# robert80203/HuPR-A-Benchmark-for-Human-Pose-Estimation-Using-Millimeter-Wave-Radar

Measured on AMD Instinct MI355X. Metric: radar frames/sec (FFT->heatmap fwd+bwd), higher is better.
Workload: dtype bf16

## Files before the change

hupr-a-benchmark-for-human-pose-estimation-using-millimeter-wave-radar_amd/csrc/attention_bf16.hip:

```cpp
#include "gemm_common.h"

namespace hupr {

constexpr float kLog2e = 1.4426950408889634f;
constexpr float kLn2 = 0.6931471805599453f;
constexpr float kDeferBits = 8.f;

typedef __bf16 bf16x8 __attribute__((ext_vector_type(8)));
typedef short s16x4 __attribute__((ext_vector_type(4)));

template <int D>
struct Img {
    static constexpr int CH = D / 8;
    static __device__ __forceinline__ int key(int row) {
        return (D == 64) ? ((((row >> 1) & 1) << 2) | ((row >> 2) & 3)) : ((((row & 3) << 2) | ((row >> 2) & 3)) | (row & (D / 8 - 1) & ~15));
    }
    static __device__ __forceinline__ int off(int row, int chunk) { return row * D + ((chunk ^ key(row)) << 3); }
};

typedef unsigned u32x4a __attribute__((ext_vector_type(4)));

template <int D, int ROWS, typename TI>
__device__ __forceinline__ void stage_rows(__bf16* img, const TI* __restrict__ src, long ld, int tid) {
    constexpr int CH = D / 8, ITEMS = ROWS * CH, PER = ITEMS / 256;
// ... 470 lines not shown
    load_frags<D, TI>(qf, Q + ((long)by * N + q) * ldq, lh);
    load_frags<D, TI>(gf, dO + ((long)by * N + q) * lddo, lh);
    const float nlse_q = -lse[(long)by * N + q] * kLog2e, d_q = Dq[(long)by * N + q];
    f32x16 nlse16;
#pragma unroll
    for (int r = 0; r < 16; ++r) nlse16[r] = nlse_q;
    f32x16 dq[D / 32];
#pragma unroll
    for (int ct = 0; ct < D / 32; ++ct)
#pragma unroll
        for (int r = 0; r < 16; ++r) dq[ct][r] = 0.f;
    constexpr bool PF = (D <= 128);
    StageRegs<PF ? D : 64, KT, TI> kr, vr;
    if (PF) {
        kr.load(K, ldk, tid);
        vr.load(V + base, D, tid);
    }
    for (int j0 = 0; j0 < N; j0 += KT) {
        __syncthreads();
        if (PF) {
            kr.store(Ks, tid);
            vr.store(Vs, tid);
        } else {
            stage_rows<D, KT, TI>(Ks, K + (long)j0 * ldk, ldk, tid);
            stage_rows<D, KT, TI>(Vs, V + base + (long)j0 * D, D, tid);
        }
        __syncthreads();
        if (PF && j0 + KT < N) {
            kr.load(K + (long)(j0 + KT) * ldk, ldk, tid);
            vr.load(V + base + (long)(j0 + KT) * D, D, tid);
        }
        f32x16 st[NT], dp[NT];
        if constexpr (QS) {
#pragma unroll
            for (int t = 0; t < NT; ++t) st[t] = nlse16;
            mma_rows_x_frags<D, false, NT>(st, Ks, qf, lr, lh);
        } else {
            mma_rows_x_frags<D, true, NT>(st, Ks, qf, lr, lh);
        }
        mma_rows_x_frags<D, true, NT>(dp, Vs, gf, lr, lh);
        {
            typedef float f32x2a __attribute__((ext_vector_type(2)));
#pragma unroll
            for (int t = 0; t < NT; ++t)
#pragma unroll
                for (int r = 0; r < 16; r += 2) {
                    const f32x2a arg = QS ? (f32x2a){st[t][r], st[t][r + 1]}
                                          : __builtin_elementwise_fma((f32x2a){st[t][r], st[t][r + 1]}, (f32x2a){kLog2e, kLog2e}, (f32x2a){nlse_q, nlse_q});
                    const f32x2a pv = {__builtin_amdgcn_exp2f(arg[0]), __builtin_amdgcn_exp2f(arg[1])};
                    const f32x2a ds = pv * ((f32x2a){dp[t][r], dp[t][r + 1]} - (f32x2a){d_q, d_q});
                    st[t][r] = ds[0];
                    st[t][r + 1] = ds[1];
                }
        }
        mma_tr_x_tile<D, D / 32, NT>(dq, Ks, st, lane);
    }
    store_ct<D>(dQ + ((long)by * N + q) * lddq, dq, 1.f, nullptr, lh);
}

template <int D, typename TI, int NH, bool QS = false>
__global__ __launch_bounds__(256, D == 64 ? 2 : 1) void hupr_k_attn_bwd_dkv(const TI* __restrict__ K, const TI* __restrict__ Q,
                                                           const TI* __restrict__ V, const TI* __restrict__ dO,
                                                           const float* dVadd,
                                                           const float* __restrict__ lse, const float* __restrict__ Dq,
                                                           float* __restrict__ dK, float* dV, int N, int ldk,
                                                           int ldq, int lddk, int lddo, const __bf16* dVadd16, int ldadd16, int xcd_map,
                                                           const AttnBwdBatch batch = AttnBwdBatch()) {
    __shared__ __attribute__((aligned(16))) __bf16 Qs[64 * D];
    __shared__ __attribute__((aligned(16))) __bf16 Gs[64 * D];
    __shared__ __attribute__((aligned(16))) float s_lse[64], s_d[64];
    const int tid = threadIdx.x, lane = tid & 63, wave = tid >> 6, lr = lane & 31, lh = lane >> 5;
    int bx, by;
    xcd_block(bx, by, xcd_map);
    if (batch.n > 0) {
        const int item = by / batch.Bn;
        by -= item * batch.Bn;
        K = static_cast<const TI*>(batch.K[item]);
        Q = static_cast<const TI*>(batch.Q[item]);
        V = static_cast<const TI*>(batch.V[item]);
        dO = static_cast<const TI*>(batch.dO[item]);
        lse = batch.lse[item];
        Dq = batch.Dq[item];
        dK = batch.dK[item];
        dV = batch.dV[item];
        dVadd = batch.add32[item];
        dVadd16 = batch.add16[item];
    }
    const long base = (long)by * N * D;
    const int key = bx * 128 + wave * 32 + lr;
    bf16x8 kf[D / 16], vf[D / 16];
    load_frags<D, TI>(kf, K + ((long)by * N + key) * ldk, lh);
    load_frags<D, TI>(vf, V + base + (long)key * D, lh);
    Q += (long)by * N * ldq;
    dO += (long)by * N * lddo;
    constexpr int DV = D / NH;
    const int c0 = blockIdx.z * DV;
    f32x16 dk[DV / 32], dv[DV / 32];
#pragma unroll
    for (int ct = 0; ct < DV / 32; ++ct)
#pragma unroll
        for (int r = 0; r < 16; ++r) { dk[ct][r] = 0.f; dv[ct][r] = 0.f; }
    constexpr bool PFQ = (D <= 128), PFG = (D == 128);
    StageRegs<PFQ ? D : 64, 64, TI> qr;
    StageRegs<PFG ? D : 64, 64, TI> gr;
    if (PFQ) qr.load(Q, ldq, tid);
    if (PFG) gr.load(dO, lddo, tid);
    for (int q0 = 0; q0 < N; q0 += 64) {
        __syncthreads();
        if (PFQ) qr.store(Qs, tid);
        else stage_rows<D, 64, TI>(Qs, Q + (long)q0 * ldq, ldq, tid);
        if (PFG) gr.store(Gs, tid);
        else stage_rows<D, 64, TI>(Gs, dO + (long)q0 * lddo, lddo, tid);
        if (tid < 64) {
            s_lse[tid] = -lse[(long)by * N + q0 + tid] * kLog2e;
            s_d[tid] = Dq[(long)by * N + q0 + tid];
        }
        __syncthreads();
        if (q0 + 64 < N) {
            if (PFQ) qr.load(Q + (long)(q0 + 64) * ldq, ldq, tid);
            if (PFG) gr.load(dO + (long)(q0 + 64) * lddo, lddo, tid);
        }
        f32x16 s[2], dp[2];
        if constexpr (QS) {
#pragma unroll
            for (int t = 0; t < 2; ++t)
#pragma unroll
                for (int r4 = 0; r4 < 4; ++r4) {
                    const float4 l4 = *reinterpret_cast<const float4*>(&s_lse[32 * t + 8 * r4 + 4 * lh]);
                    s[t][4 * r4] = l4.x; s[t][4 * r4 + 1] = l4.y; s[t][4 * r4 + 2] = l4.z; s[t][4 * r4 + 3] = l4.w;
                }
            mma_rows_x_frags<D, false>(s, Qs, kf, lr, lh);
        } else {
            mma_rows_x_frags<D>(s, Qs, kf, lr, lh);
        }
        mma_rows_x_frags<D>(dp, Gs, vf, lr, lh);
#pragma unroll
        for (int t = 0; t < 2; ++t)
#pragma unroll
            for (int r = 0; r < 16; ++r) {
                const int qi = 32 * t + (r & 3) + 8 * (r >> 2) + 4 * lh;
                const float pv = __builtin_amdgcn_exp2f(QS ? s[t][r] : fmaf(s[t][r], kLog2e, s_lse[qi]));
                dp[t][r] = pv * (dp[t][r] - s_d[qi]);
                s[t][r] = pv;
            }
        mma_tr_x_tile<D, DV / 32>(dv, Gs, s, lane, c0 / 32);
        mma_tr_x_tile<D, DV / 32>(dk, Qs, dp, lane, c0 / 32);
    }
    store_ct<DV>(dK + ((long)by * N + key) * lddk + c0, dk, QS ? kLn2 : 1.f, nullptr, lh);
    if (dVadd16) store_ct_add16<DV>(dV + base + (long)key * D + c0, dv, dVadd16 + ((long)by * N + key) * ldadd16 + c0, lh);
    else store_ct<DV>(dV + base + (long)key * D + c0, dv, 1.f, dVadd ? dVadd + base + (long)key * D + c0 : nullptr, lh);
}


template <bool QS>
__global__ __launch_bounds__(512) void hupr_k_attn_bwd_dkv512(const __bf16* __restrict__ K, const __bf16* __restrict__ Q,
                                                              const __bf16* __restrict__ V, const __bf16* __restrict__ dO,
                                                              const float* dVadd, const float* __restrict__ lse,
                                                              const float* __restrict__ Dq, float* __restrict__ dK, float* dV, int N,
                                                              int ldk, int ldq, int lddk, int lddo, const __bf16* dVadd16,
                                                              int ldadd16, int xcd_map) {
    constexpr int D = 64;
    __shared__ __attribute__((aligned(16))) __bf16 Qs[2][64 * D];
    __shared__ __attribute__((aligned(16))) __bf16 Gs[2][64 * D];
    __shared__ __attribute__((aligned(16))) float s_lse[2][64], s_d[2][64];
    const int tid = threadIdx.x, lane = tid & 63, wave = tid >> 6, lr = lane & 31, lh = lane >> 5;
    int bx, by;
    xcd_block(bx, by, xcd_map);
    const long base = (long)by * N * D;
    const int key = bx * 256 + wave * 32 + lr;
    bf16x8 kf[D / 16], vf[D / 16];
    load_frags<D, __bf16>(kf, K + ((long)by * N + key) * ldk, lh);
    load_frags<D, __bf16>(vf, V + base + (long)key * D, lh);
    Q += (long)by * N * ldq;
    dO += (long)by * N * lddo;
    f32x16 dk[D / 32], dv[D / 32];
#pragma unroll
    for (int ct = 0; ct < D / 32; ++ct)
#pragma unroll
        for (int r = 0; r < 16; ++r) { dk[ct][r] = 0.f; dv[ct][r] = 0.f; }
    const int srow = tid >> 3, sch = tid & 7;
    const __bf16* qp = Q + (long)srow * ldq + sch * 8;
    const __bf16* gp = dO + (long)srow * lddo + sch * 8;
    const float* sp = tid < 64 ? lse + (long)by * N + tid : Dq + (long)by * N + (tid & 63);
    u32x4a qreg = *reinterpret_cast<const u32x4a*>(qp), greg = *reinterpret_cast<const u32x4a*>(gp);
    float sreg = tid < 128 ? *sp : 0.f;
    *reinterpret_cast<u32x4a*>(&Qs[0][Img<D>::off(srow, sch)]) = qreg;
    *reinterpret_cast<u32x4a*>(&Gs[0][Img<D>::off(srow, sch)]) = greg;
    if (tid < 64) s_lse[0][tid] = -sreg * kLog2e;
    else if (tid < 128) s_d[0][tid - 64] = sreg;
    __syncthreads();
    for (int q0 = 0; q0 < N; q0 += 64) {
        const int cb = (q0 >> 6) & 1;
        if (q0 + 64 < N) {
            qreg = *reinterpret_cast<const u32x4a*>(qp + (long)(q0 + 64) * ldq);
            greg = *reinterpret_cast<const u32x4a*>(gp + (long)(q0 + 64) * lddo);
            if (tid < 128) sreg = sp[q0 + 64];
        }
        f32x16 s[2], dp[2];
        if constexpr (QS) {
#pragma unroll
            for (int t = 0; t < 2; ++t)
#pragma unroll
                for (int r4 = 0; r4 < 4; ++r4) {
                    const float4 l4 = *reinterpret_cast<const float4*>(&s_lse[cb][32 * t + 8 * r4 + 4 * lh]);
                    s[t][4 * r4] = l4.x; s[t][4 * r4 + 1] = l4.y; s[t][4 * r4 + 2] = l4.z; s[t][4 * r4 + 3] = l4.w;
                }
            mma_rows_x_frags<D, false>(s, Qs[cb], kf, lr, lh);
        } else {
            mma_rows_x_frags<D>(s, Qs[cb], kf, lr, lh);
        }
        mma_rows_x_frags<D>(dp, Gs[cb], vf, lr, lh);
        typedef float f32x2a __attribute__((ext_vector_type(2)));
#pragma unroll
        for (int t = 0; t < 2; ++t)
#pragma unroll
            for (int r = 0; r < 16; r += 2) {
                const int qi = 32 * t + (r & 3) + 8 * (r >> 2) + 4 * lh;
                const f32x2a dd = *reinterpret_cast<const f32x2a*>(&s_d[cb][qi]);
                f32x2a arg = {s[t][r], s[t][r + 1]};
                if constexpr (!QS) arg = __builtin_elementwise_fma(arg, (f32x2a){kLog2e, kLog2e}, *reinterpret_cast<const f32x2a*>(&s_lse[cb][qi]));
                const f32x2a pv = {__builtin_amdgcn_exp2f(arg[0]), __builtin_amdgcn_exp2f(arg[1])};
                const f32x2a ds = pv * ((f32x2a){dp[t][r], dp[t][r + 1]} - dd);
                dp[t][r] = ds[0];
                dp[t][r + 1] = ds[1];
                s[t][r] = pv[0];
                s[t][r + 1] = pv[1];
            }
        mma_tr_x_tile<D, D / 32>(dv, Gs[cb], s, lane, 0);
        mma_tr_x_tile<D, D / 32>(dk, Qs[cb], dp, lane, 0);
        if (q0 + 64 < N) {
            *reinterpret_cast<u32x4a*>(&Qs[cb ^ 1][Img<D>::off(srow, sch)]) = qreg;
            *reinterpret_cast<u32x4a*>(&Gs[cb ^ 1][Img<D>::off(srow, sch)]) = greg;
            if (tid < 64) s_lse[cb ^ 1][tid] = -sreg * kLog2e;
            else if (tid < 128) s_d[cb ^ 1][tid - 64] = sreg;
        }
        __syncthreads();
    }
    store_ct<D>(dK + ((long)by * N + key) * lddk, dk, QS ? kLn2 : 1.f, nullptr, lh);
    if (dVadd16) store_ct_add16<D>(dV + base + (long)key * D, dv, dVadd16 + ((long)by * N + key) * ldadd16, lh);
    else store_ct<D>(dV + base + (long)key * D, dv, 1.f, dVadd ? dVadd + base + (long)key * D : nullptr, lh);
}

typedef float v2fa __attribute__((ext_vector_type(2)));
constexpr int kPPRing = 8, kPPAhead = 4;

__device__ __forceinline__ void pp_dma(unsigned m0val, int voff, u32x4a rsrc, int soff) {
    unsigned keep;
    m0val = __builtin_amdgcn_readfirstlane(m0val);
    soff = __builtin_amdgcn_readfirstlane(soff);
    asm volatile("s_mov_b32 %0, m0\n\ts_mov_b32 m0, %1\n\ts_nop 0\n\tbuffer_load_dwordx4 %2, %3, %4 offen lds\n\ts_mov_b32 m0, %0"
                 : "=&s"(keep)
                 : "s"(m0val), "v"(voff), "s"(rsrc), "s"(soff)
                 : "memory");
}
#define HUPR_PP_VMCNT(N_) __builtin_amdgcn_s_waitcnt(0x0F70 | ((N_) & 15) | (((N_) >> 4) << 14))
#define HUPR_PP_BARRIER()                    \
    __builtin_amdgcn_sched_barrier(0);       \
    __builtin_amdgcn_s_barrier();            \
    __builtin_amdgcn_sched_barrier(0)

__device__ __forceinline__ u32x4a pp_rsrc(const void* base, long bytes) {
    return (u32x4a){(unsigned)(unsigned long)base, (unsigned)((unsigned long)base >> 32) & 0xffffu, (unsigned)bytes, 0x00020000u};
}

__device__ __forceinline__ void pp_block(int nqb, int Bn, int& b, int& qb) {
    const int L = blockIdx.x;
    if (Bn % 8 == 0) {
        const int idx = L >> 3;
        qb = idx % nqb;
        b = (L & 7) + 8 * (idx / nqb);
    } else {
        qb = L % nqb;
        b = L / nqb;
    }
}

template <bool QS = false>
__global__ __launch_bounds__(512, 1) void hupr_k_attn_fwd_pp64(const __bf16* __restrict__ K, const __bf16* __restrict__ Q,
                                                              const __bf16* __restrict__ V, const float* __restrict__ Vres,
                                                              float* __restrict__ out, float* __restrict__ lse, int N, int Bn, int ldk,
                                                              int ldq, __bf16* __restrict__ out16, int ld16,
                                                              unsigned long long* __restrict__ trace) {
    constexpr int D = 64;
    __shared__ __attribute__((aligned(1024))) __bf16 ring[kPPRing][2][64 * D];
    const bool tracing = trace != nullptr && blockIdx.x == 0 && (threadIdx.x >> 6) % 4 == 0;
    unsigned long long* tr = trace + (threadIdx.x >> 8) * 4096;
    int tslot = 0;
#define HUPR_PP_STAMP()                                                             \
    if (tracing) {                                                                  \
        const unsigned long long t__ = __builtin_amdgcn_s_memtime();                \
        if ((threadIdx.x & 63) == 0 && tslot < 4096) tr[tslot] = t__;               \
        ++tslot;                                                                    \
    }
    const int tid = threadIdx.x, lane = tid & 63, wave = tid >> 6, lr = lane & 31, lh = lane >> 5;
    const int grp = wave >> 2;
    if (grp == 0) __builtin_amdgcn_s_setprio(1);
    int b, qb;
    pp_block(N / 256, Bn, b, qb);
    const long base = (long)b * N * D;
    const int q = qb * 256 + wave * 32 + lr;
    const int nt = N / 64;
    bf16x8 qf[4];
    load_frags<D, __bf16>(qf, Q + ((long)b * N + q) * ldq, lh);

    const int prow = 8 * wave + (lane >> 3);
    const int pchunk = (lane & 7) ^ Img<D>::key(prow);
    const int kvoff = (prow * ldk + pchunk * 8) * 2, vvoff = (prow * D + pchunk * 8) * 2;
    const u32x4a krs = pp_rsrc(K + (long)b * N * ldk, (long)N * ldk * 2), vrs = pp_rsrc(V + base, (long)N * D * 2);
    const unsigned lds0 = (unsigned)(unsigned long)(__attribute__((address_space(3))) void*)&ring[0][0][0];
    const unsigned piece = __builtin_amdgcn_readfirstlane(lds0 + wave * 1024);
#define HUPR_PP_ISSUE(TILE_)                                                                    \
    {                                                                                           \
        const int tl_ = min((TILE_), nt - 1), sl_ = (TILE_) & (kPPRing - 1);                    \
        pp_dma(piece + sl_ * 16384, kvoff, krs, tl_ * 64 * ldk * 2);                            \
        pp_dma(piece + sl_ * 16384 + 8192, vvoff, vrs, tl_ * 64 * D * 2);                       \
    }
    int koff[4];
#pragma unroll
    for (int ks = 0; ks < 4; ++ks) koff[ks] = Img<D>::off(lr, 2 * ks + lh);
    const int g = lane >> 4, s16 = lane & 15, h = g >> 1;
    const int col = 16 * (g & 1) + 4 * (s16 & 3), rsub = s16 >> 2;
    int voff0[2], voff1[2];
#pragma unroll
    for (int ct = 0; ct < 2; ++ct) {
        const int c = 32 * ct + col;
        voff0[ct] = Img<D>::off(4 * h + rsub, c >> 3) + (c & 4);
        voff1[ct] = Img<D>::off(4 * h + rsub + 8, c >> 3) + (c & 4);
    }

    f32x16 o[2], st[2][2];
#pragma unroll
    for (int ct = 0; ct < 2; ++ct)
#pragma unroll
        for (int r = 0; r < 16; ++r) o[ct][r] = 0.f;
    float m_run = QS ? 0.f : -INFINITY, l_run = 0.f;
    f32x16 negm16 = {0.f, 0.f, 0.f, 0.f, 0.f, 0.f, 0.f, 0.f, 0.f, 0.f, 0.f, 0.f, 0.f, 0.f, 0.f, 0.f};
    bf16x8 kf[2][4], vf[2][2][2], pb[2][2][2];

#define HUPR_PP_READ_K(SLOT_)                                                                                      \
    {                                                                                                              \
        const __bf16* ki_ = &ring[SLOT_][0][0];                                                                    \
        _Pragma("unroll") for (int ks = 0; ks < 4; ++ks)                                                           \
            _Pragma("unroll") for (int t = 0; t < 2; ++t)                                                          \
                kf[t][ks] = *reinterpret_cast<const bf16x8*>(ki_ + koff[ks] + t * 32 * D);                         \
    }
#define HUPR_PP_READ_V(SLOT_)                                                                                      \
    {                                                                                                              \
        const __bf16* vi_ = &ring[SLOT_][1][0];                                                                    \
        _Pragma("unroll") for (int t = 0; t < 2; ++t)                                                              \
            _Pragma("unroll") for (int u = 0; u < 2; ++u)                                                          \
                _Pragma("unroll") for (int ct = 0; ct < 2; ++ct) {                                                 \
                    const s16x4 lo_ = __builtin_amdgcn_ds_read_tr16_b64_v4i16(                                     \
                        (__attribute__((address_space(3))) s16x4*)(vi_ + voff0[ct] + (32 * t + 16 * u) * D));     \
                    const s16x4 hi_ = __builtin_amdgcn_ds_read_tr16_b64_v4i16(                                     \
                        (__attribute__((address_space(3))) s16x4*)(vi_ + voff1[ct] + (32 * t + 16 * u) * D));     \
                    union { struct { s16x4 a, b; } s2; bf16x8 v; } uu_;                                            \
                    uu_.s2.a = lo_;                                                                                \
                    uu_.s2.b = hi_;                                                                                \
                    vf[t][u][ct] = uu_.v;                                                                          \
                }                                                                                                  \
    }
#define HUPR_PP_S(DST_)                                                                                            \
    {                                                                                                              \
        _Pragma("unroll") for (int t = 0; t < 2; ++t)                                                              \
            _Pragma("unroll") for (int r = 0; r < 16; ++r) st[DST_][t][r] = 0.f;                                   \
        _Pragma("unroll") for (int ks = 0; ks < 4; ++ks)                                                           \
            _Pragma("unroll") for (int t = 0; t < 2; ++t)                                                          \
                st[DST_][t] = __builtin_amdgcn_mfma_f32_32x32x16_bf16(kf[t][ks], qf[ks], st[DST_][t], 0, 0, 0);    \
    }
#define HUPR_PP_PV(SRC_)                                                                                           \
    _Pragma("unroll") for (int t = 0; t < 2; ++t)                                                                  \
        _Pragma("unroll") for (int u = 0; u < 2; ++u)                                                              \
            _Pragma("unroll") for (int ct = 0; ct < 2; ++ct)                                                       \
                o[ct] = __builtin_amdgcn_mfma_f32_32x32x16_bf16(vf[t][u][ct], pb[SRC_][t][u], o[ct], 0, 0, 0);

    HUPR_PP_ISSUE(0)
    HUPR_PP_ISSUE(1)
    HUPR_PP_ISSUE(2)
    HUPR_PP_ISSUE(3)
    HUPR_PP_VMCNT(4);
    HUPR_PP_BARRIER();
    HUPR_PP_READ_K(0)
    HUPR_PP_S(0)

#define HUPR_SB() __builtin_amdgcn_sched_barrier(0)
#define HUPR_PVM(T_, U_, CT_)                                                                                              \
    if (!(FIRST__)) o[CT_] = __builtin_amdgcn_mfma_f32_32x32x16_bf16(vf[T_][U_][CT_], pb[NXT__][T_][U_], o[CT_], 0, 0, 0);
#define HUPR_SM(KS_, T_)                                                                                                   \
    if (!(LAST__)) {                                                                                        \
        asm volatile("" : "+v"(kf[T_][KS_]));                                                                              \
        if ((KS_) == 0) st[NXT__][T_] = __builtin_amdgcn_mfma_f32_32x32x16_bf16(kf[T_][0], qf[0], QS ? negm16 : zero16, 0, 0, 0); \
        else st[NXT__][T_] = __builtin_amdgcn_mfma_f32_32x32x16_bf16(kf[T_][KS_], qf[KS_], st[NXT__][T_], 0, 0, 0);        \
        asm volatile("" : "+v"(kf[T_][KS_]));                                                                              \
    }
#define HUPR_M3(A_, B_, C_) fmaxf(fmaxf(A_, B_), C_)
#define HUPR_PAIR(P_)                                                                                                      \
    {                                                                                                                      \
        constexpr int t_ = (P_) >> 3, u_ = ((P_) >> 2) & 1, i_ = 2 * ((P_) & 3);                                           \
        v2fa s2_ = {st[CUR__][t_][8 * u_ + i_], st[CUR__][t_][8 * u_ + i_ + 1]};                                           \
        asm volatile("" : "+v"(s2_));                                                                                      \
        const v2fa e2_ = QS ? s2_ : __builtin_elementwise_fma(s2_, l2e2, nm2);                                             \
        const float p0_ = __builtin_amdgcn_exp2f(e2_.x);                                                         \
        const float p1_ = __builtin_amdgcn_exp2f(e2_.y);                                                         \
        sum2[(P_) & 1] += (v2fa){p0_, p1_};                                                                                \
        pb[CUR__][t_][u_][i_] = (__bf16)p0_;                                                                               \
        pb[CUR__][t_][u_][i_ + 1] = (__bf16)p1_;                                                                           \
        if (((P_) & 1) == 1) asm volatile("" : "+v"(sum2[0]), "+v"(sum2[1]));                                              \
    }
    const f32x16 zero16 = {0.f, 0.f, 0.f, 0.f, 0.f, 0.f, 0.f, 0.f, 0.f, 0.f, 0.f, 0.f, 0.f, 0.f, 0.f, 0.f};
#define HUPR_PP_TILE(CUR_, NXT_, FIRST_, LAST_)                                                                            \
    {                                                                                                                      \
        constexpr int CUR__ = CUR_, NXT__ = NXT_;                                                                          \
        constexpr bool FIRST__ = FIRST_, LAST__ = LAST_;                                                                   \
        HUPR_PP_STAMP()                                                                                                    \
        { HUPR_PP_ISSUE(j + kPPAhead) }                                                                           \
        if (!LAST__) { HUPR_PP_READ_K             ((j + 1) & (kPPRing - 1)) }                                             \
        HUPR_SB();                                                                                                         \
                          \
        const f32x16& s0_ = st[CUR__][0];                                                                                  \
        const f32x16& s1_ = st[CUR__][1];                                                                                  \
        float ma_, mb_, mc_, md_;                                                                                          \
        HUPR_PVM(0, 0, 0) ma_ = HUPR_M3(s0_[0], s0_[1], s0_[2]); mb_ = HUPR_M3(s0_[8], s0_[9], s0_[10]); HUPR_SB();        \
        HUPR_PVM(0, 0, 1) mc_ = HUPR_M3(s1_[0], s1_[1], s1_[2]); md_ = HUPR_M3(s1_[8], s1_[9], s1_[10]); HUPR_SB();        \
        HUPR_PVM(0, 1, 0) ma_ = HUPR_M3(ma_, s0_[3], s0_[4]); mb_ = HUPR_M3(mb_, s0_[11], s0_[12]); HUPR_SB();             \
        HUPR_PVM(0, 1, 1) mc_ = HUPR_M3(mc_, s1_[3], s1_[4]); md_ = HUPR_M3(md_, s1_[11], s1_[12]); HUPR_SB();             \
        HUPR_PVM(1, 0, 0) ma_ = HUPR_M3(ma_, s0_[5], s0_[6]); mb_ = HUPR_M3(mb_, s0_[13], s0_[14]); HUPR_SB();             \
        HUPR_PVM(1, 0, 1) mc_ = HUPR_M3(mc_, s1_[5], s1_[6]); md_ = HUPR_M3(md_, s1_[13], s1_[14]); HUPR_SB();             \
// ... 174 lines not shown
            HUPR_PP_FWD();
#undef HUPR_PP_FWD
            HUPR_LAUNCH_OK("hupr_k_attn_fwd_pp64");
            return HUPR_OK;
        }
    }
    if (plan_fwd(route) == HUPR_ATTN_FWD_SPLIT) {
        HUPR_REQUIRE(ws_bytes >= hupr_attn_fwd_split_ws_bytes(Bn, N, C), "%s: workspace too small", who);
        const long rows = (long)Bn * N;
        float* part_o = static_cast<float*>(ws);
        float* part_ml = part_o + (long)S * rows * C;
        grid.z = S;
        const dim3 cgrid((unsigned)((rows * (C / 4) + 255) / 256));
        hipStream_t s = as_stream(stream);
#define HUPR_ATTN_SPLIT(D_)                                                                                                \
        HUPR_LAUNCH((hupr_k_attn_fwd<D_, TI, true, QS>), grid, dim3(256), 0, s, K, Q, V, Vres, out, lse, N, ldk, ldq, o16, ld16, \
                           part_o, part_ml, AttnBatch());                                                                  \
        HUPR_LAUNCH((hupr_k_attn_combine<D_, QS>), cgrid, dim3(256), 0, s, part_o, part_ml, S, rows, Vres, out, lse, o16, ld16, AttnBatch());
        if (C == 64) { HUPR_ATTN_SPLIT(64) } else if (C == 128) { HUPR_ATTN_SPLIT(128) } else { HUPR_ATTN_SPLIT(256) }
#undef HUPR_ATTN_SPLIT
        HUPR_LAUNCH_OK("hupr_k_attn_fwd (split)");
        return HUPR_OK;
    }
    if (C == 64) HUPR_LAUNCH((hupr_k_attn_fwd<64, TI, false, QS>), grid, dim3(256), 0, as_stream(stream), K, Q, V, Vres, out, lse, N, ldk, ldq, o16, ld16, np, np, AttnBatch());
    else if (C == 128) HUPR_LAUNCH((hupr_k_attn_fwd<128, TI, false, QS>), grid, dim3(256), 0, as_stream(stream), K, Q, V, Vres, out, lse, N, ldk, ldq, o16, ld16, np, np, AttnBatch());
    else HUPR_LAUNCH((hupr_k_attn_fwd<256, TI, false, QS>), grid, dim3(256), 0, as_stream(stream), K, Q, V, Vres, out, lse, N, ldk, ldq, o16, ld16, np, np, AttnBatch());
    HUPR_LAUNCH_OK("hupr_k_attn_fwd");
    return HUPR_OK;
}

extern "C" int hupr_attn_fwd_bf16(const float* K, const float* Q, const float* V, float* out, float* lse, int Bn, int N, int C,
                                  int residual, hupr_stream_t stream) {
    return attn_fwd("hupr_attn_fwd_bf16", K, C, Q, C, V, residual ? V : nullptr, out, lse, nullptr, 0, Bn, N, C, stream);
}
extern "C" int hupr_attn_fwd_bf16in(const void* K, const void* Q, const void* V, const float* Vres, float* out, float* lse,
                                    int Bn, int N, int C, hupr_stream_t stream) {
    return attn_fwd("hupr_attn_fwd_bf16in", static_cast<const __bf16*>(K), C, static_cast<const __bf16*>(Q), C,
                    static_cast<const __bf16*>(V), Vres, out, lse, nullptr, 0, Bn, N, C, stream);
}
extern "C" int hupr_attn_fwd_bf16in_ld(const void* K, int ldk, const void* Q, int ldq, const void* V, const float* Vres,
                                       float* out, float* lse, void* out16, int ld16, int Bn, int N, int C,
                                       hupr_stream_t stream) {
    return attn_fwd("hupr_attn_fwd_bf16in_ld", static_cast<const __bf16*>(K), ldk, static_cast<const __bf16*>(Q), ldq,
                    static_cast<const __bf16*>(V), Vres, out, lse, out16, ld16, Bn, N, C, stream);
}
template <bool QS>
static int attn_fwd_batch(const char* who, const hupr_attn_item* items, int n_items, int ldk, int ldq, int ld16, int Bn, int N,
                          int C, void* ws, size_t ws_bytes, hupr_stream_t stream) {
    HUPR_REQUIRE(items && n_items >= 1 && n_items <= 4 && Bn > 0, "%s: bad argument", who);
    HUPR_REQUIRE(hupr_attn_flash_supported(N, C), "%s: unsupported shape N=%d C=%d", who, N, C);
    HUPR_REQUIRE(ldk >= C && ldq >= C && ldk % 8 == 0 && ldq % 8 == 0, "%s: bad row strides %d %d", who, ldk, ldq);
    const int route = attn_plan(Bn, N, C, ldk, true, ws != nullptr);
    HUPR_REQUIRE(route > 0, "%s: bad argument", who);
    const int S = plan_splits(route);
    bool any16 = false;
    for (int i = 0; i < n_items; ++i) {
        HUPR_REQUIRE(items[i].K && items[i].Q && items[i].V && items[i].out && items[i].lse, "%s: null pointer in item %d", who, i);
        any16 = any16 || items[i].out16;
    }
    HUPR_REQUIRE(!any16 || (ld16 >= C && ld16 % 4 == 0), "%s: bad bf16 output stride %d", who, ld16);
    if (plan_fwd(route) == HUPR_ATTN_FWD_PP64) {
        for (int i = 0; i < n_items; ++i) {
            const int rc = attn_fwd<__bf16, QS>(who, static_cast<const __bf16*>(items[i].K), ldk, static_cast<const __bf16*>(items[i].Q), ldq,
                                               static_cast<const __bf16*>(items[i].V), items[i].Vres, items[i].out, items[i].lse,
                                               items[i].out16, ld16, Bn, N, C, stream);
            if (rc) return rc;
        }
        return HUPR_OK;
    }
    HUPR_REQUIRE(S == 1 || ws_bytes >= (size_t)n_items * hupr_attn_fwd_split_ws_bytes(Bn, N, C), "%s: workspace too small", who);
    AttnBatch b = AttnBatch();
    b.n = n_items;
    b.splits = S;
    for (int i = 0; i < n_items; ++i) {
        b.K[i] = items[i].K; b.Q[i] = items[i].Q; b.V[i] = items[i].V; b.Vres[i] = items[i].Vres;
        b.out[i] = items[i].out; b.lse[i] = items[i].lse; b.out16[i] = static_cast<__bf16*>(items[i].out16);
    }
    if (plan_fwd(route) == HUPR_ATTN_FWD_ONE_PASS) {
        const dim3 g1(N / 128, Bn, n_items);
        hipStream_t s1 = as_stream(stream);
        const __bf16* const k0 = nullptr;
        float* const f0 = nullptr;
        __bf16* const h0 = nullptr;
        if (C == 64) HUPR_LAUNCH((hupr_k_attn_fwd<64, __bf16, false, QS>), g1, dim3(256), 0, s1, k0, k0, k0, f0, f0, f0, N, ldk, ldq, h0, ld16, f0, f0, b);
        else if (C == 128) HUPR_LAUNCH((hupr_k_attn_fwd<128, __bf16, false, QS>), g1, dim3(256), 0, s1, k0, k0, k0, f0, f0, f0, N, ldk, ldq, h0, ld16, f0, f0, b);
        else HUPR_LAUNCH((hupr_k_attn_fwd<256, __bf16, false, QS>), g1, dim3(256), 0, s1, k0, k0, k0, f0, f0, f0, N, ldk, ldq, h0, ld16, f0, f0, b);
        HUPR_LAUNCH_OK("hupr_k_attn_fwd (batch)");
        return HUPR_OK;
    }
    const long rows = (long)Bn * N;
    float* part_o = static_cast<float*>(ws);
    float* part_ml = part_o + (long)n_items * S * rows * C;
    const dim3 grid(N / 128, Bn, S * n_items);
    const dim3 cgrid((unsigned)((rows * (C / 4) + 255) / 256), n_items);
    hipStream_t s = as_stream(stream);
    typedef __bf16 TI;
    const TI* const nk = nullptr;
    float* const nf = nullptr;
    __bf16* const nh = nullptr;
#define HUPR_ATTN_BATCH(D_)                                                                                                          \
    HUPR_LAUNCH((hupr_k_attn_fwd<D_, TI, true, QS>), grid, dim3(256), 0, s, nk, nk, nk, nf, nf, nf, N, ldk, ldq, nh, ld16, part_o, part_ml, b); \
    HUPR_LAUNCH((hupr_k_attn_combine<D_, QS>), cgrid, dim3(256), 0, s, part_o, part_ml, S, rows, nf, nf, nf, nh, ld16, b);
    if (C == 64) { HUPR_ATTN_BATCH(64) } else if (C == 128) { HUPR_ATTN_BATCH(128) } else { HUPR_ATTN_BATCH(256) }
#undef HUPR_ATTN_BATCH
    HUPR_LAUNCH_OK("hupr_k_attn_fwd (split, batch)");
    return HUPR_OK;
}
extern "C" int hupr_attn_fwd_bf16in_ld_ws_batch(const hupr_attn_item* items, int n_items, int ldk, int ldq, int ld16, int Bn, int N,
                                                int C, void* ws, size_t ws_bytes, hupr_stream_t stream) {
    return attn_fwd_batch<false>("hupr_attn_fwd_bf16in_ld_ws_batch", items, n_items, ldk, ldq, ld16, Bn, N, C, ws, ws_bytes, stream);
}
extern "C" int hupr_attn_fwd_bf16in_ld_ws_batch_qs(const hupr_attn_item* items, int n_items, int ldk, int ldq, int ld16, int Bn, int N,
                                                   int C, void* ws, size_t ws_bytes, hupr_stream_t stream) {
    return attn_fwd_batch<true>("hupr_attn_fwd_bf16in_ld_ws_batch_qs", items, n_items, ldk, ldq, ld16, Bn, N, C, ws, ws_bytes, stream);
}

extern "C" int hupr_attn_fwd_bf16in_ld_ws(const void* K, int ldk, const void* Q, int ldq, const void* V, const float* Vres,
                                          float* out, float* lse, void* out16, int ld16, int Bn, int N, int C, void* ws,
                                          size_t ws_bytes, hupr_stream_t stream) {
    return attn_fwd("hupr_attn_fwd_bf16in_ld_ws", static_cast<const __bf16*>(K), ldk, static_cast<const __bf16*>(Q), ldq,
                    static_cast<const __bf16*>(V), Vres, out, lse, out16, ld16, Bn, N, C, stream, ws, ws_bytes);
}
extern "C" int hupr_attn_fwd_bf16in_ld_ws_qs(const void* K, int ldk, const void* Qs, int ldq, const void* V, const float* Vres,
                                             float* out, float* lse, void* out16, int ld16, int Bn, int N, int C, void* ws,
                                             size_t ws_bytes, hupr_stream_t stream) {
    return attn_fwd<__bf16, true>("hupr_attn_fwd_bf16in_ld_ws_qs", static_cast<const __bf16*>(K), ldk, static_cast<const __bf16*>(Qs), ldq,
                                  static_cast<const __bf16*>(V), Vres, out, lse, out16, ld16, Bn, N, C, stream, ws, ws_bytes);
}

template <typename TI, bool QS = false>
static int attn_bwd(const char* who, const TI* K, int ldk, const TI* Q, int ldq, const TI* V, const TI* dO, int lddo,
                    const float* V32, const float* out, const float* dout32, const float* lse, float* dK, int lddk, float* dQ,
                    int lddq, float* dV, int accumulate, float* Dq, int Bn, int N, int C, int residual, hupr_stream_t stream) {
    HUPR_REQUIRE(K && Q && V && dO && V32 && out && lse && dK && dQ && dV && Dq && Bn > 0, "%s: bad argument", who);
    HUPR_REQUIRE(dout32 || sizeof(TI) == 2, "%s: fp32 operands need the fp32 gradient", who);
    HUPR_REQUIRE(hupr_attn_flash_supported(N, C), "%s: unsupported shape N=%d C=%d", who, N, C);
    HUPR_REQUIRE(ldk >= C && ldq >= C && lddk >= C && lddq >= C && lddo >= C && ldk % 8 == 0 && ldq % 8 == 0 && lddo % 8 == 0 &&
                     lddk % 4 == 0 && lddq % 4 == 0,
                 "%s: bad row strides", who);
    HUPR_REQUIRE(!(residual && accumulate), "%s: accumulate is for the non-residual form", who);
    const int route = attn_plan(Bn, N, C, ldk, sizeof(TI) == 2, false);
    HUPR_REQUIRE(route > 0, "%s: bad argument", who);
    hipStream_t s = as_stream(stream);
    const long rows = (long)Bn * N;
    dim3 grid(N / 128, Bn);
    const float* add32 = residual ? dout32 : (accumulate ? dV : nullptr);
    const __bf16* add16 = (residual && !dout32) ? reinterpret_cast<const __bf16*>(dO) : nullptr;
    const dim3 pgrid((unsigned)((rows + 15) / 16));
    const int xmap = plan_xmap(route);
    const bool dkv512 = plan_dkv(route) == HUPR_ATTN_DKV512;
#define HUPR_ATTN_BWD(D_, NH_)                                                                                             \
    if (dout32) HUPR_LAUNCH((hupr_k_attn_prep<D_, float>), pgrid, dim3(256), 0, s, dout32, C, out, V32, Dq, rows, residual); \
    else HUPR_LAUNCH((hupr_k_attn_prep<D_, __bf16>), pgrid, dim3(256), 0, s, reinterpret_cast<const __bf16*>(dO), lddo, out, V32, Dq, rows, residual); \
    HUPR_LAUNCH((hupr_k_attn_bwd_dq<D_, TI, QS>), grid, dim3(256), 0, s, K, Q, V, dO, lse, Dq, dQ, N, ldk, ldq, lddq, lddo, xmap);  \
    if (dkv512)                                                                                                              \
        HUPR_LAUNCH(hupr_k_attn_bwd_dkv512<QS>, dim3(N / 256, Bn), dim3(512), 0, s, reinterpret_cast<const __bf16*>(K),       \
                           reinterpret_cast<const __bf16*>(Q), reinterpret_cast<const __bf16*>(V), reinterpret_cast<const __bf16*>(dO), \
                           add32, lse, Dq, dK, dV, N, ldk, ldq, lddk, lddo, add16, lddo, xmap);                                 \
    else                                                                                                                     \
        HUPR_LAUNCH((hupr_k_attn_bwd_dkv<D_, TI, NH_, QS>), dim3(N / 128, Bn, NH_), dim3(256), 0, s, K, Q, V, dO, add32, lse, Dq, \
                           dK, dV, N, ldk, ldq, lddk, lddo, add16, lddo, xmap);
    if (C == 64) { HUPR_ATTN_BWD(64, 1) } else if (C == 128) { HUPR_ATTN_BWD(128, 1) } else { HUPR_ATTN_BWD(256, 2) }
#undef HUPR_ATTN_BWD
    HUPR_LAUNCH_OK("hupr_k_attn_bwd");
    return HUPR_OK;
}

template <bool QS>
static int attn_bwd_batch(const char* who, const hupr_attn_bwd_item* items, int n_items, int ldk, int ldq, int lddo, int lddk, int lddq,
                          int Bn, int N, int C, hupr_stream_t stream) {
    HUPR_REQUIRE(items && n_items >= 1 && n_items <= 4 && Bn > 0, "%s: bad argument", who);
    HUPR_REQUIRE(hupr_attn_flash_supported(N, C), "%s: unsupported shape N=%d C=%d", who, N, C);
    for (int i = 0; i < n_items; ++i) {
        const hupr_attn_bwd_item& t = items[i];
        HUPR_REQUIRE(t.K && t.Q && t.V && t.dO && t.V32 && t.out && t.lse && t.dK && t.dQ && t.dV && t.Dq, "%s: null pointer in item %d", who, i);
        HUPR_REQUIRE(!(t.residual && t.accumulate), "%s: accumulate is for the non-residual form (item %d)", who, i);
    }
    const int route = attn_plan(Bn, N, C, ldk, true, false);
    HUPR_REQUIRE(route > 0, "%s: bad row strides", who);
    const bool level1 = plan_dkv(route) == HUPR_ATTN_DKV512;
    if (n_items == 1) {
        for (int i = 0; i < n_items; ++i) {
            const hupr_attn_bwd_item& t = items[i];
            const int rc = attn_bwd<__bf16, QS>(who, static_cast<const __bf16*>(t.K), ldk, static_cast<const __bf16*>(t.Q), ldq,
                                               static_cast<const __bf16*>(t.V), static_cast<const __bf16*>(t.dO), lddo, t.V32, t.out, nullptr,
                                               t.lse, t.dK, lddk, t.dQ, lddq, t.dV, t.accumulate, t.Dq, Bn, N, C, t.residual, stream);
            if (rc) return rc;
        }
        return HUPR_OK;
    }
    HUPR_REQUIRE(ldk >= C && ldq >= C && lddk >= C && lddq >= C && lddo >= C && ldk % 8 == 0 && ldq % 8 == 0 && lddo % 8 == 0 &&
                     lddk % 4 == 0 && lddq % 4 == 0, "%s: bad row strides", who);
    hipStream_t s = as_stream(stream);
    const long rows = (long)Bn * N;
    const int xmap = plan_xmap(route);
    AttnBwdBatch b = AttnBwdBatch();
    b.n = n_items;
    b.Bn = Bn;
    for (int i = 0; i < n_items; ++i) {
        const hupr_attn_bwd_item& t = items[i];
        b.K[i] = t.K; b.Q[i] = t.Q; b.V[i] = t.V; b.dO[i] = t.dO; b.out[i] = t.out; b.V32[i] = t.V32; b.lse[i] = t.lse;
        b.Dq[i] = t.Dq; b.dK[i] = t.dK; b.dQ[i] = t.dQ; b.dV[i] = t.dV; b.residual[i] = t.residual;
        b.add32[i] = t.accumulate ? t.dV : nullptr;
        b.add16[i] = t.residual ? static_cast<const __bf16*>(t.dO) : nullptr;
    }
    const __bf16* const k0 = nullptr;
    const float* const c0 = nullptr;
    float* const f0 = nullptr;
    const dim3 pgrid((unsigned)((rows + 15) / 16), n_items), qgrid(N / 128, Bn * n_items);
    int round_of[4], n_rounds = 0;
    for (int i = 0; i < n_items; ++i) {
        int r = 0;
        for (int j = 0; j < i; ++j)
            if (items[j].dV == items[i].dV) r = round_of[j] + 1 > r ? round_of[j] + 1 : r;
        round_of[i] = r;
        n_rounds = r + 1 > n_rounds ? r + 1 : n_rounds;
    }
#define HUPR_ATTN_BWD_BATCH(D_, NH_)                                                                                             \
    HUPR_LAUNCH((hupr_k_attn_prep<D_, __bf16>), pgrid, dim3(256), 0, s, k0, lddo, c0, c0, f0, rows, 0, b);                      \
    HUPR_LAUNCH((hupr_k_attn_bwd_dq<D_, __bf16, QS>), qgrid, dim3(256), 0, s, k0, k0, k0, k0, c0, c0, f0, N, ldk, ldq, lddq, lddo, xmap, b); \
    for (int r = 0; r < n_rounds; ++r) {                                                                                         \
        AttnBwdBatch br = AttnBwdBatch();                                                                                        \
        br.Bn = Bn;                                                                                                              \
        for (int i = 0; i < n_items; ++i)                                                                                        \
            if (round_of[i] == r) {                                                                                              \
                const int k = br.n++;                                                                                            \
                br.K[k] = b.K[i]; br.Q[k] = b.Q[i]; br.V[k] = b.V[i]; br.dO[k] = b.dO[i]; br.lse[k] = b.lse[i]; br.Dq[k] = b.Dq[i]; \
                br.dK[k] = b.dK[i]; br.dV[k] = b.dV[i]; br.add32[k] = b.add32[i]; br.add16[k] = b.add16[i];                      \
            }                                                                                                                    \
        HUPR_LAUNCH((hupr_k_attn_bwd_dkv<D_, __bf16, NH_, QS>), dim3(N / 128, Bn * br.n, NH_), dim3(256), 0, s, k0, k0, k0, k0, c0, c0, c0, \
                    f0, f0, N, ldk, ldq, lddk, lddo, k0, lddo, xmap, br);                                                        \
    }
    if (level1) {
        HUPR_LAUNCH((hupr_k_attn_prep<64, __bf16>), pgrid, dim3(256), 0, s, k0, lddo, c0, c0, f0, rows, 0, b);
        HUPR_LAUNCH((hupr_k_attn_bwd_dq<64, __bf16, QS>), qgrid, dim3(256), 0, s, k0, k0, k0, k0, c0, c0, f0, N, ldk, ldq, lddq, lddo, xmap, b);
        for (int i = 0; i < n_items; ++i)
            HUPR_LAUNCH(hupr_k_attn_bwd_dkv512<QS>, dim3(N / 256, Bn), dim3(512), 0, s, static_cast<const __bf16*>(b.K[i]),
                        static_cast<const __bf16*>(b.Q[i]), static_cast<const __bf16*>(b.V[i]), static_cast<const __bf16*>(b.dO[i]), b.add32[i],
                        b.lse[i], b.Dq[i], b.dK[i], b.dV[i], N, ldk, ldq, lddk, lddo, b.add16[i], lddo, xmap);
    } else if (C == 64) { HUPR_ATTN_BWD_BATCH(64, 1) } else if (C == 128) { HUPR_ATTN_BWD_BATCH(128, 1) } else { HUPR_ATTN_BWD_BATCH(256, 2) }
#undef HUPR_ATTN_BWD_BATCH
    HUPR_LAUNCH_OK("hupr_k_attn_bwd (batch)");
    return HUPR_OK;
}
extern "C" int hupr_attn_bwd_bf16in_ld_batch(const hupr_attn_bwd_item* items, int n_items, int ldk, int ldq, int lddo, int lddk,
                                             int lddq, int Bn, int N, int C, hupr_stream_t stream) {
    return attn_bwd_batch<false>("hupr_attn_bwd_bf16in_ld_batch", items, n_items, ldk, ldq, lddo, lddk, lddq, Bn, N, C, stream);
}
extern "C" int hupr_attn_bwd_bf16in_ld_batch_qs(const hupr_attn_bwd_item* items, int n_items, int ldk, int ldq, int lddo, int lddk,
                                                int lddq, int Bn, int N, int C, hupr_stream_t stream) {
    return attn_bwd_batch<true>("hupr_attn_bwd_bf16in_ld_batch_qs", items, n_items, ldk, ldq, lddo, lddk, lddq, Bn, N, C, stream);
}

extern "C" int hupr_attn_bwd_bf16(const float* K, const float* Q, const float* V, const float* out, const float* dout,
                                  const float* lse, float* dK, float* dQ, float* dV, float* Dq, int Bn, int N, int C,
                                  int residual, hupr_stream_t stream) {
    return attn_bwd("hupr_attn_bwd_bf16", K, C, Q, C, V, dout, C, V, out, dout, lse, dK, C, dQ, C, dV, 0, Dq, Bn, N, C, residual,
                    stream);
}
extern "C" int hupr_attn_bwd_bf16in(const void* K, const void* Q, const void* V, const void* dO, const float* V32,
                                    const float* out, const float* dout32, const float* lse, float* dK, float* dQ, float* dV,
                                    float* Dq, int Bn, int N, int C, int residual, hupr_stream_t stream) {
    HUPR_REQUIRE(dout32, "hupr_attn_bwd_bf16in: null pointer");
    return attn_bwd("hupr_attn_bwd_bf16in", static_cast<const __bf16*>(K), C, static_cast<const __bf16*>(Q), C,
                    static_cast<const __bf16*>(V), static_cast<const __bf16*>(dO), C, V32, out, dout32, lse, dK, C, dQ, C, dV, 0,
                    Dq, Bn, N, C, residual, stream);
}
extern "C" int hupr_attn_bwd_bf16in_ld(const void* K, int ldk, const void* Q, int ldq, const void* V, const void* dO, int lddo,
                                       const float* V32, const float* out, const float* dout32, const float* lse, float* dK,
                                       int lddk, float* dQ, int lddq, float* dV, float* Dq, int Bn, int N, int C,
                                       int residual, int accumulate, hupr_stream_t stream) {
    return attn_bwd("hupr_attn_bwd_bf16in_ld", static_cast<const __bf16*>(K), ldk, static_cast<const __bf16*>(Q), ldq,
                    static_cast<const __bf16*>(V), static_cast<const __bf16*>(dO), lddo, V32, out, dout32, lse, dK, lddk, dQ,
                    lddq, dV, accumulate, Dq, Bn, N, C, residual, stream);
}
extern "C" int hupr_attn_bwd_bf16in_ld_qs(const void* K, int ldk, const void* Qs, int ldq, const void* V, const void* dO, int lddo,
                                          const float* V32, const float* out, const float* dout32, const float* lse, float* dK,
                                          int lddk, float* dQ, int lddq, float* dV, float* Dq, int Bn, int N, int C,
                                          int residual, int accumulate, hupr_stream_t stream) {
    return attn_bwd<__bf16, true>("hupr_attn_bwd_bf16in_ld_qs", static_cast<const __bf16*>(K), ldk, static_cast<const __bf16*>(Qs), ldq,
                                  static_cast<const __bf16*>(V), static_cast<const __bf16*>(dO), lddo, V32, out, dout32, lse, dK, lddk,
                                  dQ, lddq, dV, accumulate, Dq, Bn, N, C, residual, stream);
}
```

Baseline: 1791.

## Add software-pipelined dQ backward kernel with async LDS DMA ring for D=64

Adds a 512-thread dQ backward attention kernel for head dim 64 that streams K/V tiles into an 8-deep LDS ring with buffer_load-to-LDS DMA issued four tiles ahead. It interleaves the score/dP MFMAs of the next tile with the softmax-gradient math of the current tile, using scheduling group barriers. It replaces the older 256-thread dQ kernel on the dkv512 and level1 batch paths. The goal is to hide global load latency and keep the matrix units busy, at the cost of a large LDS footprint, one block per CU, and reliance on hand-tuned scheduling.

Result: no change. 1793, median of 6 (+0.1%).

```diff
diff --git a/hupr-a-benchmark-for-human-pose-estimation-using-millimeter-wave-radar_amd/csrc/attention_bf16.hip b/hupr-a-benchmark-for-human-pose-estimation-using-millimeter-wave-radar_amd/csrc/attention_bf16.hip
--- a/hupr-a-benchmark-for-human-pose-estimation-using-millimeter-wave-radar_amd/csrc/attention_bf16.hip
+++ b/hupr-a-benchmark-for-human-pose-estimation-using-millimeter-wave-radar_amd/csrc/attention_bf16.hip
@@ -646,6 +646,40 @@
 }
 
 
+typedef float v2fa __attribute__((ext_vector_type(2)));
+constexpr int kPPRing = 8, kPPAhead = 4;
+
+__device__ __forceinline__ void pp_dma(unsigned m0val, int voff, u32x4a rsrc, int soff) {
+    unsigned keep;
+    m0val = __builtin_amdgcn_readfirstlane(m0val);
+    soff = __builtin_amdgcn_readfirstlane(soff);
+    asm volatile("s_mov_b32 %0, m0\n\ts_mov_b32 m0, %1\n\ts_nop 0\n\tbuffer_load_dwordx4 %2, %3, %4 offen lds\n\ts_mov_b32 m0, %0"
+                 : "=&s"(keep)
+                 : "s"(m0val), "v"(voff), "s"(rsrc), "s"(soff)
+                 : "memory");
+}
+#define HUPR_PP_VMCNT(N_) __builtin_amdgcn_s_waitcnt(0x0F70 | ((N_) & 15) | (((N_) >> 4) << 14))
+#define HUPR_PP_BARRIER()                    \
+    __builtin_amdgcn_sched_barrier(0);       \
+    __builtin_amdgcn_s_barrier();            \
+    __builtin_amdgcn_sched_barrier(0)
+
+__device__ __forceinline__ u32x4a pp_rsrc(const void* base, long bytes) {
+    return (u32x4a){(unsigned)(unsigned long)base, (unsigned)((unsigned long)base >> 32) & 0xffffu, (unsigned)bytes, 0x00020000u};
+}
+
+__device__ __forceinline__ void pp_block(int nqb, int Bn, int& b, int& qb) {
+    const int L = blockIdx.x;
+    if (Bn % 8 == 0) {
+        const int idx = L >> 3;
+        qb = idx % nqb;
+        b = (L & 7) + 8 * (idx / nqb);
+    } else {
+        qb = L % nqb;
+        b = L / nqb;
+    }
+}
+
 template <bool QS>
 __global__ __launch_bounds__(512) void hupr_k_attn_bwd_dkv512(const __bf16* __restrict__ K, const __bf16* __restrict__ Q,
                                                               const __bf16* __restrict__ V, const __bf16* __restrict__ dO,
@@ -735,38 +769,123 @@
     else store_ct<D>(dV + base + (long)key * D, dv, 1.f, dVadd ? dVadd + base + (long)key * D : nullptr, lh);
 }
 
-typedef float v2fa __attribute__((ext_vector_type(2)));
-constexpr int kPPRing = 8, kPPAhead = 4;
-
-__device__ __forceinline__ void pp_dma(unsigned m0val, int voff, u32x4a rsrc, int soff) {
-    unsigned keep;
-    m0val = __builtin_amdgcn_readfirstlane(m0val);
-    soff = __builtin_amdgcn_readfirstlane(soff);
-    asm volatile("s_mov_b32 %0, m0\n\ts_mov_b32 m0, %1\n\ts_nop 0\n\tbuffer_load_dwordx4 %2, %3, %4 offen lds\n\ts_mov_b32 m0, %0"
-                 : "=&s"(keep)
-                 : "s"(m0val), "v"(voff), "s"(rsrc), "s"(soff)
-                 : "memory");
-}
-#define HUPR_PP_VMCNT(N_) __builtin_amdgcn_s_waitcnt(0x0F70 | ((N_) & 15) | (((N_) >> 4) << 14))
-#define HUPR_PP_BARRIER()                    \
-    __builtin_amdgcn_sched_barrier(0);       \
-    __builtin_amdgcn_s_barrier();            \
-    __builtin_amdgcn_sched_barrier(0)
-
-__device__ __forceinline__ u32x4a pp_rsrc(const void* base, long bytes) {
-    return (u32x4a){(unsigned)(unsigned long)base, (unsigned)((unsigned long)base >> 32) & 0xffffu, (unsigned)bytes, 0x00020000u};
-}
-
-__device__ __forceinline__ void pp_block(int nqb, int Bn, int& b, int& qb) {
-    const int L = blockIdx.x;
-    if (Bn % 8 == 0) {
-        const int idx = L >> 3;
-        qb = idx % nqb;
-        b = (L & 7) + 8 * (idx / nqb);
-    } else {
-        qb = L % nqb;
-        b = L / nqb;
-    }
+template <bool QS>
+__global__ __launch_bounds__(512, 1) void hupr_k_attn_bwd_dq_pp64(const __bf16* __restrict__ K, const __bf16* __restrict__ Q,
+                                                                 const __bf16* __restrict__ V, const __bf16* __restrict__ dO,
+                                                                 const float* __restrict__ lse, const float* __restrict__ Dq,
+                                                                 float* __restrict__ dQ, int N, int ldk, int ldq, int lddq, int lddo,
+                                                                 int xcd_map, const AttnBwdBatch batch) {
+    constexpr int D = 64;
+    __shared__ __attribute__((aligned(1024))) __bf16 ring[kPPRing][2][64 * D];
+    const int tid = threadIdx.x, lane = tid & 63, wave = tid >> 6, lr = lane & 31, lh = lane >> 5;
+    int bx, by;
+    xcd_block(bx, by, xcd_map);
+    if (batch.n > 0) {
+        const int item = by / batch.Bn;
+        by -= item * batch.Bn;
+        K = static_cast<const __bf16*>(batch.K[item]);
+        Q = static_cast<const __bf16*>(batch.Q[item]);
+        V = static_cast<const __bf16*>(batch.V[item]);
+        dO = static_cast<const __bf16*>(batch.dO[item]);
+        lse = batch.lse[item];
+        Dq = batch.Dq[item];
+        dQ = batch.dQ[item];
+    }
+    const long base = (long)by * N * D;
+    const int q = bx * 256 + wave * 32 + lr;
+    const int nt = N / 64;
+    bf16x8 qf[D / 16], gf[D / 16];
+    load_frags<D, __bf16>(qf, Q + ((long)by * N + q) * ldq, lh);
+    load_frags<D, __bf16>(gf, dO + ((long)by * N + q) * lddo, lh);
+    const float nlse_q = -lse[(long)by * N + q] * kLog2e, d_q = Dq[(long)by * N + q];
+    f32x16 nlse16;
+#pragma unroll
+    for (int r = 0; r < 16; ++r) nlse16[r] = nlse_q;
+    f32x16 dq[D / 32];
+#pragma unroll
+    for (int ct = 0; ct < D / 32; ++ct)
+#pragma unroll
+        for (int r = 0; r < 16; ++r) dq[ct][r] = 0.f;
+    const int prow = 8 * wave + (lane >> 3);
+    const int pchunk = (lane & 7) ^ Img<D>::key(prow);
+    const int kvoff = (prow * ldk + pchunk * 8) * 2, vvoff = (prow * D + pchunk * 8) * 2;
+    const __bf16* Kb = K + (long)by * N * ldk;
+    const u32x4a vrs = pp_rsrc(V + base, (long)N * D * 2);
+    const unsigned lds0 = (unsigned)(unsigned long)(__attribute__((address_space(3))) void*)&ring[0][0][0];
+    const unsigned piece = __builtin_amdgcn_readfirstlane(lds0 + wave * 1024);
+    auto issue = [&](int tile) {
+        const int tl = min(tile, nt - 1), sl = tile & (kPPRing - 1);
+        pp_dma(piece + sl * 16384, kvoff, pp_rsrc(Kb + (long)tl * 64 * ldk, 64L * ldk * 2), 0);
+        pp_dma(piece + sl * 16384 + 8192, vvoff, vrs, tl * 64 * D * 2);
+    };
+    typedef float f32x2a __attribute__((ext_vector_type(2)));
+    auto sdp = [&](f32x16* st, f32x16* dp, int sl) {
+        const __bf16* Ks = &ring[sl][0][0];
+        const __bf16* Vs = &ring[sl][1][0];
+#pragma unroll
+        for (int t = 0; t < 2; ++t) {
+#pragma unroll
+            for (int r = 0; r < 16; ++r) {
+                st[t][r] = QS ? nlse_q : 0.f;
+                dp[t][r] = 0.f;
+            }
+        }
+#pragma unroll
+        for (int ks = 0; ks < 4; ++ks)
+#pragma unroll
+            for (int t = 0; t < 2; ++t)
+                st[t] = __builtin_amdgcn_mfma_f32_32x32x16_bf16(*reinterpret_cast<const bf16x8*>(&Ks[Img<D>::off(32 * t + lr, 2 * ks + lh)]),
+                                                                 qf[ks], st[t], 0, 0, 0);
+#pragma unroll
+        for (int ks = 0; ks < 4; ++ks)
+#pragma unroll
+            for (int t = 0; t < 2; ++t)
+                dp[t] = __builtin_amdgcn_mfma_f32_32x32x16_bf16(*reinterpret_cast<const bf16x8*>(&Vs[Img<D>::off(32 * t + lr, 2 * ks + lh)]),
+                                                                 gf[ks], dp[t], 0, 0, 0);
+    };
+    auto dsv = [&](f32x16* st, const f32x16* dp) {
+#pragma unroll
+        for (int t = 0; t < 2; ++t)
+#pragma unroll
+            for (int r = 0; r < 16; r += 2) {
+                const f32x2a arg = QS ? (f32x2a){st[t][r], st[t][r + 1]}
+                                      : __builtin_elementwise_fma((f32x2a){st[t][r], st[t][r + 1]}, (f32x2a){kLog2e, kLog2e}, (f32x2a){nlse_q, nlse_q});
+                const f32x2a pv = {__builtin_amdgcn_exp2f(arg[0]), __builtin_amdgcn_exp2f(arg[1])};
+                const f32x2a ds = pv * ((f32x2a){dp[t][r], dp[t][r + 1]} - (f32x2a){d_q, d_q});
+                st[t][r] = ds[0];
+                st[t][r + 1] = ds[1];
+            }
+    };
+    auto tile = [&](f32x16* st_c, f32x16* dp_c, f32x16* st_n, f32x16* dp_n, int j) {
+        issue(j + kPPAhead);
+        __builtin_amdgcn_sched_barrier(0);
+        sdp(st_n, dp_n, (j + 1) & (kPPRing - 1));
+        dsv(st_c, dp_c);
+        __builtin_amdgcn_sched_group_barrier(0x100, 2, 0);
+#pragma unroll
+        for (int i_ = 0; i_ < 14; ++i_) {
+            __builtin_amdgcn_sched_group_barrier(0x008, 1, 0);
+            __builtin_amdgcn_sched_group_barrier(0x100, 1, 0);
+            __builtin_amdgcn_sched_group_barrier(0x002, 5, 0);
+        }
+        __builtin_amdgcn_sched_group_barrier(0x008, 2, 0);
+        __builtin_amdgcn_sched_barrier(0);
+        mma_tr_x_tile<D, D / 32>(dq, &ring[j & (kPPRing - 1)][0][0], st_c, lane);
+        HUPR_PP_VMCNT(2 * kPPAhead - 4);
+        HUPR_PP_BARRIER();
+    };
+#pragma unroll
+    for (int i = 0; i < kPPAhead; ++i) issue(i);
+    HUPR_PP_VMCNT(2 * kPPAhead - 4);
+    HUPR_PP_BARRIER();
+    f32x16 sa[2], da[2], sb[2], db[2];
+    sdp(sa, da, 0);
+    for (int j = 0; j < nt; j += 2) {
+        tile(sa, da, sb, db, j);
+        tile(sb, db, sa, da, j + 1);
+    }
+    HUPR_PP_VMCNT(0);
+    store_ct<D>(dQ + ((long)by * N + q) * lddq, dq, 1.f, nullptr, lh);
 }
 
 template <bool QS = false>
@@ -1247,7 +1366,12 @@
 #define HUPR_ATTN_BWD(D_, NH_)                                                                                             \
     if (dout32) HUPR_LAUNCH((hupr_k_attn_prep<D_, float>), pgrid, dim3(256), 0, s, dout32, C, out, V32, Dq, rows, residual); \
     else HUPR_LAUNCH((hupr_k_attn_prep<D_, __bf16>), pgrid, dim3(256), 0, s, reinterpret_cast<const __bf16*>(dO), lddo, out, V32, Dq, rows, residual); \
-    HUPR_LAUNCH((hupr_k_attn_bwd_dq<D_, TI, QS>), grid, dim3(256), 0, s, K, Q, V, dO, lse, Dq, dQ, N, ldk, ldq, lddq, lddo, xmap);  \
+    if (dkv512)                                                                                                              \
+        HUPR_LAUNCH(hupr_k_attn_bwd_dq_pp64<QS>, dim3(N / 256, Bn), dim3(512), 0, s, reinterpret_cast<const __bf16*>(K),        \
+                           reinterpret_cast<const __bf16*>(Q), reinterpret_cast<const __bf16*>(V), reinterpret_cast<const __bf16*>(dO), \
+                           lse, Dq, dQ, N, ldk, ldq, lddq, lddo, xmap, AttnBwdBatch());                                        \
+    else                                                                                                                     \
+        HUPR_LAUNCH((hupr_k_attn_bwd_dq<D_, TI, QS>), grid, dim3(256), 0, s, K, Q, V, dO, lse, Dq, dQ, N, ldk, ldq, lddq, lddo, xmap); \
     if (dkv512)                                                                                                              \
         HUPR_LAUNCH(hupr_k_attn_bwd_dkv512<QS>, dim3(N / 256, Bn), dim3(512), 0, s, reinterpret_cast<const __bf16*>(K),       \
                            reinterpret_cast<const __bf16*>(Q), reinterpret_cast<const __bf16*>(V), reinterpret_cast<const __bf16*>(dO), \
@@ -1328,7 +1452,8 @@
     }
     if (level1) {
         HUPR_LAUNCH((hupr_k_attn_prep<64, __bf16>), pgrid, dim3(256), 0, s, k0, lddo, c0, c0, f0, rows, 0, b);
-        HUPR_LAUNCH((hupr_k_attn_bwd_dq<64, __bf16, QS>), qgrid, dim3(256), 0, s, k0, k0, k0, k0, c0, c0, f0, N, ldk, ldq, lddq, lddo, xmap, b);
+        HUPR_LAUNCH(hupr_k_attn_bwd_dq_pp64<QS>, dim3(N / 256, Bn * n_items), dim3(512), 0, s, k0, k0, k0, k0, c0, c0, f0, N, ldk, ldq, lddq,
+                    lddo, xmap, b);
         for (int i = 0; i < n_items; ++i)
             HUPR_LAUNCH(hupr_k_attn_bwd_dkv512<QS>, dim3(N / 256, Bn), dim3(512), 0, s, static_cast<const __bf16*>(b.K[i]),
                         static_cast<const __bf16*>(b.Q[i]), static_cast<const __bf16*>(b.V[i]), static_cast<const __bf16*>(b.dO[i]), b.add32[i],
```
